# lzzcd001/MeshDiffusion

Hardware: NVIDIA H100
Metric: denoising sample-steps/sec at res-64 (4x64^3), uncond_gen PC sampler (higher is better)
Workload: dtype bf16x3

## Files before the change

meshdiffusion_b200/csrc/gemm_host.cu:

```cuda
#include "gemm_host.h"
#include "elementwise.cuh"
#include <cstring>
#include <cstdlib>
#include <mutex>

namespace mdb {

typedef CUresult (*PFN_encodeTiled)(CUtensorMap*, CUtensorMapDataType, cuuint32_t, void*, const cuuint64_t*,
                                    const cuuint64_t*, const cuuint32_t*, const cuuint32_t*, CUtensorMapInterleave,
                                    CUtensorMapSwizzle, CUtensorMapL2promotion, CUtensorMapFloatOOBfill);

static PFN_encodeTiled get_encode() {
  static PFN_encodeTiled fn = nullptr;
  static std::once_flag once;
  std::call_once(once, [] {
    void* f = nullptr;
    cudaDriverEntryPointQueryResult q;
    cudaError_t e = cudaGetDriverEntryPoint("cuTensorMapEncodeTiled", &f, cudaEnableDefault, &q);
    if (e != cudaSuccess || q != cudaDriverEntryPointSuccess || !f)
      throw std::runtime_error("mdb: cuTensorMapEncodeTiled not available (needs an sm_90+ driver)");
    fn = reinterpret_cast<PFN_encodeTiled>(f);
  });
  return fn;
}
// ... 193 lines not shown
  p.ocs = 1;
  p.kb_elems = kb_elems(prec);
}

void GemmOp::set_output(Precision pr, int X, int Y, int Z, int B, int N, void* out, long long ldc, bool out_fp32) {
  set_output_strided(pr, X, Y, Z, B, N, out, ldc, ldc * X, ldc * X * Y, ldc * X * Y * Z, out_fp32);
}

MapDesc act_map(const Act& a, Precision prec, int part, Geometry box, int sub, int px, int py, int pz) {
  const long long es = esize(prec);
  const long long sx = a.row() * parts(prec) * es, sy = sx * a.X, sz = sy * a.Y, sb = sz * a.Z;
  MapDesc m;
  m.rank = 5;
  m.base = static_cast<char*>(a.ptr) + (long long)part * a.row() * es + px * sx + py * sy + pz * sz;
  m.dims[0] = a.C; m.dims[1] = (a.X - px + sub - 1) / sub; m.dims[2] = (a.Y - py + sub - 1) / sub;
  m.dims[3] = (a.Z - pz + sub - 1) / sub; m.dims[4] = a.B;
  m.strides[0] = sx * sub; m.strides[1] = sy * sub; m.strides[2] = sz * sub; m.strides[3] = sb;
  m.box[0] = kb_elems(prec); m.box[1] = box.bx; m.box[2] = box.by; m.box[3] = box.bz; m.box[4] = box.bb;
  return m;
}

int GemmOp::add_amap(const Act& a, int halo, int sub, int px, int py, int pz, int part) {
  if ((int)amaps_.size() >= kMaxAMaps) throw std::runtime_error("mdb: too many A tensor maps");
  if (halo > 0 && (geo.bz != 1 || geo.bb != 1)) throw std::runtime_error("mdb: halo needs a (bx,by,1,1) tile");
  amaps_.push_back(act_map(a, prec, part, {geo.bx, geo.by + halo, geo.bz, geo.bb}, sub, px, py, pz));
  return (int)amaps_.size() - 1;
}

void GemmOp::add_load_x(int tm_hi, int tm_lo, int nk, int rows, int jrows, int dx, int dy, int dz, int c0, int wsrc,
                        int wc0, int tap0, int tapj) {
  if ((int)loads.size() >= kMaxLoads) throw std::runtime_error("mdb: load table overflow");
  if (rows > kAStageRows) throw std::runtime_error("mdb: A box exceeds the stage size");
  LoadEntry e{};
  e.tmap = (uint8_t)tm_hi; e.tmap_lo = (uint8_t)(prec == kBF16X3 ? tm_lo : tm_hi);
  e.nk = (uint8_t)nk; e.rows = (uint8_t)rows; e.jrows = (uint8_t)jrows;
  e.dx = (int8_t)dx; e.dy = (int8_t)dy; e.dz = (int8_t)dz; e.wsrc = (uint8_t)wsrc;
  e.c0 = (uint16_t)c0; e.wc0 = (uint16_t)wc0; e.tap0 = (uint8_t)tap0; e.tapj = (uint8_t)tapj;
  loads.push_back(e);
  ksteps += nk;
}

void GemmOp::add_conv(const std::vector<Act>& srcs, const float* w, int k, int stride) {
  int ctot = 0;
  for (auto& s : srcs) ctot += s.C;
  const int T = k * k * k;
  add_conv_w(srcs, WSrc{w, 1LL * ctot * T, (long long)T, 1, ctot}, k, stride);
}

void GemmOp::add_conv_dgrad(const Act& dy, const float* w_oidhw, int cin_total, int k) {
  const int T = k * k * k;
  add_conv_w({dy}, WSrc{w_oidhw + (T - 1), (long long)T, 1LL * cin_total * T, -1, dy.C}, k, 1);
}

void GemmOp::add_conv_w(const std::vector<Act>& srcs, const WSrc& wsrc, int k, int stride) {
  const int KB = kb_elems(prec);
  int ctot = 0;
  for (auto& s : srcs) ctot += s.C;
  const int T = k * k * k;
  const int ws = add_wsrc(wsrc);
  const int pad = k / 2;
  flops += 2.0 * p.X * p.Y * p.Z * p.Bn * (double)p.N * ctot * T;
  int coff = 0;
  if (stride == 1) {
    const bool reuse = geo.bz == 1 && geo.bb == 1 && geo.bx * (geo.by + k - 1) <= kAStageRows && p.Y >= geo.by;
    const bool x3 = prec == kBF16X3;
    for (auto& s : srcs) {
      const int tm = add_amap(s, reuse ? k - 1 : 0);
      const int tl = x3 ? add_amap(s, reuse ? k - 1 : 0, 1, 0, 0, 0, 1) : tm;
      for (int c0 = 0; c0 < s.C; c0 += KB) {
        if (reuse) {
          for (int dz = 0; dz < k; ++dz)
            for (int dx = 0; dx < k; ++dx)
              add_load_x(tm, tl, k, geo.bx * (geo.by + k - 1), geo.bx, dx - pad, -pad, dz - pad, c0, ws, coff + c0,
                         (dz * k) * k + dx, k);
        } else {
          for (int dz = 0; dz < k; ++dz)
            for (int dy = 0; dy < k; ++dy)
              for (int dx = 0; dx < k; ++dx)
                add_load_x(tm, tl, 1, kBlockM, 0, dx - pad, dy - pad, dz - pad, c0, ws, coff + c0, (dz * k + dy) * k + dx, 0);
        }
      }
      coff += s.C;
    }
  } else if (stride == 2) {
    if (k != 3) throw std::runtime_error("mdb: stride-2 conv supports k=3 only");
    const bool x3 = prec == kBF16X3;
    for (auto& s : srcs) {
      int tm[8], tl[8];
      for (int par = 0; par < 8; ++par) tm[par] = add_amap(s, 0, 2, par & 1, (par >> 1) & 1, (par >> 2) & 1);
      for (int par = 0; par < 8; ++par) tl[par] = x3 ? add_amap(s, 0, 2, par & 1, (par >> 1) & 1, (par >> 2) & 1, 1) : tm[par];
      for (int c0 = 0; c0 < s.C; c0 += KB)
        for (int dz = 0; dz < 3; ++dz)
          for (int dy = 0; dy < 3; ++dy)
            for (int dx = 0; dx < 3; ++dx) {
              const int par = (dx & 1) | ((dy & 1) << 1) | ((dz & 1) << 2);
              add_load_x(tm[par], tl[par], 1, kBlockM, 0, dx >> 1, dy >> 1, dz >> 1, c0, ws, coff + c0, (dz * 3 + dy) * 3 + dx, 0);
            }
      coff += s.C;
    }
  } else {
    throw std::runtime_error("mdb: unsupported stride");
  }
}

void GemmOp::add_conv_up2(const Act& s, const float* w8, int px, int py, int pz) {
  const int KB = kb_elems(prec);
  const int ws = add_wsrc(WSrc{w8, 8LL * s.C, 8, 1, s.C});
  flops += 2.0 * p.X * p.Y * p.Z * p.Bn * (double)p.N * s.C * 8;
  const bool x3 = prec == kBF16X3;
  const bool reuse = geo.bz == 1 && geo.bb == 1 && geo.bx * (geo.by + 1) <= kAStageRows && p.Y >= geo.by;
  const int tm = add_amap(s, reuse ? 1 : 0);
  const int tl = x3 ? add_amap(s, reuse ? 1 : 0, 1, 0, 0, 0, 1) : tm;
  for (int c0 = 0; c0 < s.C; c0 += KB) {
    for (int ez = 0; ez < 2; ++ez)
      for (int ex = 0; ex < 2; ++ex) {
        if (reuse) {
          add_load_x(tm, tl, 2, geo.bx * (geo.by + 1), geo.bx, ex - 1 + px, -1 + py, ez - 1 + pz, c0, ws, c0, (ez * 2) * 2 + ex, 2);
        } else {
          for (int ey = 0; ey < 2; ++ey)
            add_load_x(tm, tl, 1, kBlockM, 0, ex - 1 + px, ey - 1 + py, ez - 1 + pz, c0, ws, c0, (ez * 2 + ey) * 2 + ex, 0);
        }
      }
  }
}

void GemmOp::add_pointwise(const std::vector<Act>& srcs, const float* w, bool w_in_out) {
  int ctot = 0;
  for (auto& s : srcs) ctot += s.C;
  WSrc ws = w_in_out ? WSrc{w, 1, (long long)p.N, 0, ctot} : WSrc{w, (long long)ctot, 1, 0, ctot};
  add_pointwise_w(srcs, &ws);
}

void GemmOp::add_pointwise_w(const std::vector<Act>& srcs, const WSrc* w) {
  const int KB = kb_elems(prec);
  int ctot = 0;
  for (auto& s : srcs) ctot += s.C;
  int ws = 0;
  if (w) ws = add_wsrc(*w);
  flops += 2.0 * p.X * p.Y * p.Z * p.Bn * (double)p.N * ctot;
  int coff = 0;
  for (auto& s : srcs) {
    const int tm = add_amap(s, 0);
    const int tl = prec == kBF16X3 ? add_amap(s, 0, 1, 0, 0, 0, 1) : tm;
    for (int c0 = 0; c0 < s.C; c0 += KB) add_load_x(tm, tl, 1, kBlockM, 0, 0, 0, 0, c0, ws, coff + c0, 0, 0);
    coff += s.C;
  }
}

void GemmOp::set_residual(const void* res, long long ldr, long long batch_stride, bool fp32) {
  p.res = res;
  p.batch_fastest = batch_stride == 0 ? 1 : 0;
  p.rsx = ldr; p.rsy = ldr * p.X; p.rsz = ldr * p.X * p.Y; p.rsb = batch_stride;
  p.res_fp32 = fp32 ? 1 : 0;
  p.res_lo_off = physical_strides(prec == kBF16X3 && !fp32, ldr, p.rsx, p.rsy, p.rsz, p.rsb);
}

void GemmOp::set_gn_backward(const void* x0, long long ld0, int c0, const void* x1, long long ld1, const void* consts, int silu,
                             float* part) {
  if (prec == kTF32 || p.out_fp32 || p.ocs != 1)
    throw std::runtime_error("mdb: the GroupNorm-backward epilogue is built for bf16 / split-bf16 NDHWC outputs");
  if (p.N % 32 != 0 || (ld1 > 0 && c0 % 32 != 0)) throw std::runtime_error("mdb: GroupNorm-backward epilogue needs 32-channel aligned sources");
  if (splits > 1) throw std::runtime_error("mdb: GroupNorm-backward epilogue cannot be combined with split-K");
  gnb = true;
  p.res = x0; p.res_fp32 = 0; p.batch_fastest = 0;
  p.rsx = ld0; p.rsy = ld0 * p.X; p.rsz = ld0 * p.X * p.Y; p.rsb = ld0 * p.X * p.Y * p.Z;
  p.res1 = x1; p.res_c0 = ld1 > 0 ? c0 : p.N;
  p.r1sx = ld1; p.r1sy = ld1 * p.X; p.r1sz = ld1 * p.X * p.Y; p.r1sb = ld1 * p.X * p.Y * p.Z;
  p.res_lo_off = physical_strides(prec == kBF16X3, ld0, p.rsx, p.rsy, p.rsz, p.rsb);
  p.res1_lo_off = physical_strides(prec == kBF16X3, ld1, p.r1sx, p.r1sy, p.r1sz, p.r1sb);
  p.gnb_c = reinterpret_cast<const float4*>(consts);
  p.gnb_silu = silu;
  p.gnb_part = part;
}

MapDesc GemmOp::b_desc(void* ptr, long long K, int N, int batch, long long rsb, long long bsb) const {
  MapDesc m;
  m.base = ptr; m.rank = 3;
  m.dims[0] = (uint64_t)K; m.dims[1] = (uint64_t)N; m.dims[2] = (uint64_t)batch;
  m.strides[0] = (uint64_t)rsb; m.strides[1] = (uint64_t)bsb;
  m.box[0] = (uint32_t)kb_elems(prec); m.box[1] = (uint32_t)block_n; m.box[2] = 1;
  return m;
}

void GemmOp::set_b_activation(void* ptr, int K, int N, int batch, long long rs, long long bs) {
  b_from_act = true;
  p.b_batched = 1;
  const long long es = esize(prec);
  if (prec == kBF16X3) {
    if (K % kb_elems(prec) != 0) throw std::runtime_error("mdb: X3 activation-B operands need K to be a multiple of 64");
    b_lo_off = rs;
    bmap_ = b_desc(ptr, (int)(rs + K), N, batch, 2 * rs * es, 2 * bs * es);
    return;
  }
  bmap_ = b_desc(ptr, K, N, batch, rs * es, bs * es);
}

struct PackWSrc { const float* ptr; long long sn, sc, st; int cvalid; int ndiv; long long sn_hi; int cdiv; long long sc_hi; };
struct PackArgs { PackWSrc w[4]; };

template <Precision P>
__global__ void __launch_bounds__(256) pack_weights_kernel(const LoadEntry* __restrict__ loads, const int* __restrict__ load_ks0,
                                                         int n_loads, const __grid_constant__ PackArgs args, int N, int ksteps,
                                                         int KB, void* __restrict__ out) {
  const int vpk = KB >> 3;
  const long long total = 1LL * N * n_loads * vpk;
  for (long long idx = blockIdx.x * (long long)blockDim.x + threadIdx.x; idx < total; idx += (long long)gridDim.x * blockDim.x) {
    const int v8 = (int)(idx % vpk);
    const long long t = idx / vpk;
    const int l = (int)(t % n_loads);
    const int n = (int)(t / n_loads);
    const LoadEntry e = loads[l];
    const PackWSrc& w = args.w[e.wsrc];
    const long long noff = w.ndiv ? (long long)(n % w.ndiv) * w.sn + (long long)(n / w.ndiv) * w.sn_hi : (long long)n * w.sn;
    const int c0 = e.wc0 + v8 * 8;
    long long coff[8];
    unsigned valid = 0;
#pragma unroll
    for (int i = 0; i < 8; ++i) {
      const int c = c0 + i;
      if (c < w.cvalid) valid |= 1u << i;
      coff[i] = noff + (w.cdiv ? (long long)(c % w.cdiv) * w.sc + (long long)(c / w.cdiv) * w.sc_hi : (long long)c * w.sc);
    }
    const long long obase = ((long long)n * ksteps + load_ks0[l]) * parts(P) * KB + v8 * 8;
    for (int j = 0; j < e.nk; ++j) {
      const long long toff = (long long)(e.tap0 + j * e.tapj) * w.st;
      float v[8];
#pragma unroll
      for (int i = 0; i < 8; ++i) v[i] = (valid >> i) & 1u ? __ldg(w.ptr + coff[i] + toff) : 0.f;
      ActElem<P>* op = reinterpret_cast<ActElem<P>*>(out) + obase + (long long)j * parts(P) * KB;
      constexpr int E = kVecElems<P>;
#pragma unroll
      for (int i = 0; i < 8 / E; ++i) store_vec<P>(op + E * i, (long long)KB * sizeof(ActElem<P>), v + E * i);
    }
  }
}

void GemmOp::repack(cudaStream_t stream) {
  if (b_from_act) return;
  if (!d_ks0) {
    std::vector<int> ks0;
    int run = 0;
    for (size_t l = 0; l < loads.size(); ++l) { ks0.push_back(run); run += loads[l].nk; }
    if (run != ksteps) throw std::runtime_error("mdb: load table does not cover the packed K extent");
    MDB_CUDA_CHECK(cudaMalloc(&d_ks0, ks0.size() * sizeof(int)));
    MDB_CUDA_CHECK(cudaMemcpy(d_ks0, ks0.data(), ks0.size() * sizeof(int), cudaMemcpyHostToDevice));
  }
  if (wsrcs.size() > 4) throw std::runtime_error("mdb: too many weight sources");
  PackArgs args{};
  for (size_t i = 0; i < wsrcs.size(); ++i) args.w[i] = {wsrcs[i].ptr, wsrcs[i].sn, wsrcs[i].sc, wsrcs[i].st, wsrcs[i].cvalid, wsrcs[i].ndiv, wsrcs[i].sn_hi, wsrcs[i].cdiv, wsrcs[i].sc_hi};
  const int KB = kb_elems(prec), n_loads = (int)loads.size();
  const long long total = 1LL * p.N * n_loads * (KB / 8);
  int blocks = (int)((total + 255) / 256);
  if (blocks > kPlanSMs * 16) blocks = kPlanSMs * 16;
  if (prec == kTF32)
    pack_weights_kernel<kTF32><<<blocks, 256, 0, stream>>>(d_loads, d_ks0, n_loads, args, p.N, ksteps, KB, d_wpacked);
  else if (prec == kBF16X3)
    pack_weights_kernel<kBF16X3><<<blocks, 256, 0, stream>>>(d_loads, d_ks0, n_loads, args, p.N, ksteps, KB, d_wpacked);
  else
    pack_weights_kernel<kBF16><<<blocks, 256, 0, stream>>>(d_loads, d_ks0, n_loads, args, p.N, ksteps, KB, d_wpacked);
  MDB_CUDA_CHECK(cudaGetLastError());
}

void GemmOp::finalize() {
  if (loads.empty()) throw std::runtime_error("mdb: GemmOp without loads");
  p.b_explicit_k = 0;
  p.b_kstep = kb_elems(prec) * parts(prec);
  p.b_lo_k = kb_elems(prec);
  if (b_from_act) p.b_kstep = kb_elems(prec);
  if (b_from_act && prec == kBF16X3) {
    p.b_explicit_k = 1;
    p.b_lo_k = (int)b_lo_off;
  }
  if (!b_from_act) p.b_batched = 0;
  p.n_loads = (int)loads.size();
  if (p.splits < 1) p.splits = 1;
  {
    a_slot_need = 0;
    nk_max = 0;
    p.n_segs = 0;
    p.total_groups = 0;
    size_t i = 0;
    while (i < loads.size()) {
      size_t j = i;
      while (j < loads.size() && loads[j].nk == loads[i].nk && loads[j].rows == loads[i].rows && loads[j].jrows == loads[i].jrows) ++j;
      if (p.n_segs >= kMaxSegs) throw std::runtime_error("mdb: too many pipeline segments");
      GemmSeg sg{};
      sg.n_groups = (int)(j - i); sg.nk = loads[i].nk;
      sg.a_bytes = loads[i].rows * kRowBytes;
      sg.a_stride = (sg.a_bytes + 1023) / 1024 * 1024;
      sg.jbytes = loads[i].jrows * kRowBytes;
      const int need = parts(prec) * sg.a_stride;
      if (sg.a_stride > kAStageBytes) throw std::runtime_error("mdb: A box exceeds the slot size");
      if (need > a_slot_need) a_slot_need = need;
      if (sg.nk > nk_max) nk_max = sg.nk;
      p.segs[p.n_segs++] = sg;
      p.total_groups += sg.n_groups;
      i = j;
    }
  }
  if (p.splits > p.total_groups) { p.splits = p.total_groups; splits = p.splits; }
}

bool GemmOp::epi_tma_ok(const GemmParams& p) const {
  if (gnb || block_n != 128 || prec == kTF32 || p.splits > 1 || p.ocs != 1 || p.out_fp32) return false;
  if (p.res && (p.res_fp32 || p.batch_fastest)) return false;
  const long long es = esize(prec);
  auto aligned = [&](const void* base, long long lo_off, long long sx, long long sy, long long sz, long long sb) {
    const uintptr_t a = reinterpret_cast<uintptr_t>(base);
    return a % 16 == 0 && (lo_off * es) % 16 == 0 && (sx * es) % 16 == 0 && (sy * es) % 16 == 0 && (sz * es) % 16 == 0 &&
           (sb * es) % 16 == 0;
  };
  if (!aligned(p.out, prec == kBF16X3 ? p.out_lo_off : 0, p.osx, p.osy, p.osz, p.osb)) return false;
  if (p.res && !aligned(p.res, prec == kBF16X3 ? p.res_lo_off : 0, p.rsx, p.rsy, p.rsz, p.rsb)) return false;
  return true;
}

static MapDesc epi_map(const void* base, Precision prec, int part, long long lo_off, const GemmParams& q, int B, long long sx,
                       long long sy, long long sz, long long sb) {
  const long long es = esize(prec);
  MapDesc m;
  m.rank = 5;
  m.base = const_cast<char*>(static_cast<const char*>(base)) + (long long)part * lo_off * es;
  m.dims[0] = q.N; m.dims[1] = q.X; m.dims[2] = q.Y; m.dims[3] = q.Z; m.dims[4] = B;
  const long long st[4] = {sx * es, sy * es, sz * es, sb * es};
  long long prev = es * q.N;
  for (int i = 0; i < 4; ++i) {
    m.strides[i] = (uint64_t)(m.dims[i + 1] == 1 ? prev : st[i]);
    prev = (long long)m.strides[i] * (long long)m.dims[i + 1];
  }
  m.box[0] = kRowBytes / es; m.box[1] = q.bx; m.box[2] = q.by; m.box[3] = q.bz; m.box[4] = q.bb;
  return m;
}

void GemmOp::encode_epi_maps(GemmParams& q, int B) const {
  for (int part = 0; part < parts(prec); ++part) {
    encode_map(&q.omap[part], prec, epi_map(q.out, prec, part, q.out_lo_off, q, B, q.osx, q.osy, q.osz, q.osb));
    if (q.res) encode_map(&q.rmap[part], prec, epi_map(q.res, prec, part, q.res_lo_off, q, B, q.rsx, q.rsy, q.rsz, q.rsb));
  }
}

void GemmOp::upload(cudaStream_t stream) {
  for (size_t i = 0; i < amaps_.size(); ++i) encode_map(&p.amap[i], prec, amaps_[i]);
  p.epi_tma = epi_tma_ok(p) ? 1 : 0;
  if (p.epi_tma && p.out) encode_epi_maps(p, p.Bn);
#ifdef MDB_EPI_TRACE
  if (getenv("MDB_EPI_TRACE_PER_THREAD")) p.epi_tma = 0;
  MDB_CUDA_CHECK(cudaMalloc(&d_trace, sizeof(unsigned long long) * kTraceCtas * kTraceTiles * kTraceStamps));
  MDB_CUDA_CHECK(cudaMemset(d_trace, 0, sizeof(unsigned long long) * kTraceCtas * kTraceTiles * kTraceStamps));
  p.trace = d_trace;
  trace_registry().push_back(this);
#endif
  MDB_CUDA_CHECK(cudaMalloc(&d_loads, loads.size() * sizeof(LoadEntry)));
  MDB_CUDA_CHECK(cudaMemcpyAsync(d_loads, loads.data(), loads.size() * sizeof(LoadEntry), cudaMemcpyHostToDevice, stream));
  p.loads = d_loads;
  if (!b_from_act) {
    const long long ktot = 1LL * ksteps * kb_elems(prec) * parts(prec);
    const long long bytes = ktot * p.N * esize(prec);
    MDB_CUDA_CHECK(cudaMalloc(&d_wpacked, bytes));
    owns_w = true;
    bmap_ = b_desc(d_wpacked, ktot, p.N, 1, ktot * esize(prec), bytes);
  }
  encode_map(&p.bmap, prec, bmap_);
  MDB_CUDA_CHECK(cudaStreamSynchronize(stream));
}

void GemmOp::launch(cudaStream_t stream, int B, void* out_override) const {
  GemmParams p = this->p;
  const int smem = pick_slots(p);
  if (B > 0) {
    if (B > this->p.Bn) throw std::runtime_error("mdb: batch exceeds the batch the op was built for");
    p.Bn = B;
    p.tb = (B + p.bb - 1) / p.bb;
  }
  if (out_override) p.out = out_override;
  if (p.epi_tma && (out_override || p.Bn != this->p.Bn)) {
    p.epi_tma = epi_tma_ok(p) ? 1 : 0;
    if (p.epi_tma) encode_epi_maps(p, p.Bn);
  }
  const int tiles_m = p.tx * p.ty * p.tz * p.tb;
  const int total = tiles_m * p.n_tiles_n * (p.splits > 1 ? p.splits : 1);
  const int grid = total < sm_count() ? total : sm_count();
  if (gnb) {
    if (p.splits > 1) throw std::runtime_error("mdb: GroupNorm-backward epilogue: no split-K");
    p.gnb_drop_thresh = rt_drop_thresh; p.gnb_drop_scale = rt_drop_scale; p.gnb_seed = rt_seed;
  }
  gemm_variant(block_n, prec, gnb).launch(p, grid, smem, stream);
  if (p.splits > 1) {
    SplitReduceArgs a{};
    a.partial = p.partial; a.split_stride = p.split_stride; a.splits = p.splits;
    a.bias = p.bias; a.rowbias = p.rowbias; a.rowbias_ld = p.rowbias_ld;
    a.res = p.res; a.res_batch_stride = p.rsb;
    a.out = p.out; a.stats = p.stats; a.voxels = (long long)p.X * p.Y * p.Z; a.N = p.N; a.prec = prec;
    if (prec == kBF16X3) a.res_batch_stride = p.rsb / 2;
    launch_split_reduce(a, p.Bn, stream);
  }
}

}
```

meshdiffusion_b200/csrc/gemm_tc.cuh:

```cuda
#pragma once
#include "ptx.cuh"
#include "act_format.cuh"
#include "gn_stats.cuh"

namespace mdb {

constexpr int kBlockM = 128;
constexpr int kRowBytes = 128;
constexpr int kAStageRows = 160;
constexpr int kAStageBytes = kAStageRows * kRowBytes;
constexpr int kMaxLoads = 2048;
constexpr int kMaxAMaps = 16;
constexpr int kGemmThreads = 384;
constexpr int kEpiThreads = 256;

struct __align__(16) LoadEntry {
  uint8_t tmap;
  uint8_t nk;
  uint8_t rows;
  uint8_t jrows;
  int8_t dx, dy, dz;
  uint8_t wsrc;
  uint16_t c0;
  uint16_t wc0;
  uint8_t tap0;
  uint8_t tapj;
  uint8_t tmap_lo;
  uint8_t pad;
};
static_assert(sizeof(LoadEntry) == 16, "LoadEntry must be 16 bytes");

struct GemmSeg {
  int n_groups;
  int nk;
  int a_bytes;
  int a_stride;
  int jbytes;
};
constexpr int kMaxSegs = 8;

struct GemmParams {
  CUtensorMap amap[kMaxAMaps];
  CUtensorMap bmap;
  CUtensorMap omap[2];
  CUtensorMap rmap[2];
  int epi_tma;
#ifdef MDB_EPI_TRACE
  unsigned long long* trace;
#endif
  const LoadEntry* loads;
  int n_loads;
  int n_segs;
  GemmSeg segs[kMaxSegs];
  int bx, by, bz, bb;
  int X, Y, Z, Bn;
  int tx, ty, tz, tb;
  int n_tiles_n;
  int N;
  int b_batched;
  int splits;
  int total_groups;
  float* partial;
  long long split_stride;
  int batch_fastest;
  int kb_elems;
  int b_explicit_k;
  int b_kstep;
  int b_lo_k;
  int n_aslots, a_slot_bytes, n_bslots, b_slot_bytes;
  long long out_lo_off, res_lo_off;
  void* out;
  long long osx, osy, osz, osb;
  long long ocs;
  int out_fp32;
  const float* bias;
  int bias_on_m;
  const float* rowbias;
  long long rowbias_ld;
  const void* res;
  long long rsx, rsy, rsz, rsb;
  int res_fp32;
  float alpha;
  long long* stats;
  const void* res1;
  long long r1sx, r1sy, r1sz, r1sb;
  long long res1_lo_off;
  int res_c0;
  const float4* gnb_c;
  int gnb_silu;
  int gnb_drop_thresh; float gnb_drop_scale; unsigned long long gnb_seed;
  float* gnb_part;
};

constexpr int kMaxSlots = 8;
constexpr int kMaxDynSmem = 232448;
template <int BLOCK_N, bool kWholeTile = false>
struct GemmCfg {
  static constexpr int kBTileBytes = BLOCK_N * kRowBytes;
  static constexpr int kStatsFloats = 24 * BLOCK_N;
  static constexpr int kStageCols = (kWholeTile || BLOCK_N < 64) ? BLOCK_N : 64;
  static constexpr int kStageRounds = BLOCK_N / kStageCols;
  static_assert(kStageRounds <= 2, "the epilogue stages at most two rounds");
  static constexpr int kAccPitch = kStageCols + 4;
  static constexpr int kAccFloats = kBlockM * kAccPitch;
  static constexpr int kFixedBytes = 1024 + kAccFloats * 4 + kStatsFloats * 4 + 4 * kMaxSlots * 8;
};
constexpr int kRegsProducer = 40, kRegsConsumer = 232;

template <int BLOCK_N, Precision P, bool GNB>
constexpr bool kHasTmaEpi = !GNB && BLOCK_N == 128 && P != kTF32;
constexpr int kEpiBoxBytes = 64 * 2 * kBlockM;
static_assert(kEpiBoxBytes == GemmCfg<128>::kBTileBytes, "an epilogue box is one weight tile");

#ifdef MDB_EPI_TRACE
constexpr int kTraceCtas = 16, kTraceTiles = 64, kTraceStamps = 6;
#define MDB_STAMP(k) do { if (trace_row && et == 0) trace_row[k] = globaltimer(); } while (0)
#else
#define MDB_STAMP(k) do { } while (0)
#endif

__device__ __forceinline__ uint64_t kdesc(uint32_t saddr) { return make_wgmma_desc(saddr, 16, 1024); }

template <int OFF>
__device__ __forceinline__ void colsum_butterfly(float (&s)[32], float (&ss)[32], int lane) {
  const bool hi = (lane & OFF) != 0;
#pragma unroll
  for (int i = 0; i < OFF; ++i) {
    const float send_s = hi ? s[i] : s[i + OFF];
    const float send_q = hi ? ss[i] : ss[i + OFF];
    const float keep_s = hi ? s[i + OFF] : s[i];
    const float keep_q = hi ? ss[i + OFF] : ss[i];
    s[i] = keep_s + __shfl_xor_sync(0xffffffffu, send_s, OFF);
    ss[i] = keep_q + __shfl_xor_sync(0xffffffffu, send_q, OFF);
  }
  if constexpr (OFF > 1) colsum_butterfly<OFF / 2>(s, ss, lane);
}

template <Precision P>
__device__ __forceinline__ void add_res_chunk(const uint4 (&buf)[8], float (&v)[32]) {
  constexpr int E = kVecElems<P>, NV = 32 / E;
#pragma unroll
  for (int i = 0; i < NV; ++i) {
    float r[E];
    decode_vec<P>(buf[i], buf[P == kBF16X3 ? NV + i : i], r);
#pragma unroll
    for (int j = 0; j < E; ++j) v[E * i + j] += r[j];
  }
}

template <int BLOCK_N, Precision P, bool GNB>
__global__ void __launch_bounds__(kGemmThreads, 1) gemm_tc_kernel(const __grid_constant__ GemmParams p) {
  static_assert(!(GNB && P == kTF32), "the GroupNorm-backward epilogue is built for bf16 / split-bf16 operands");
  using Cfg = GemmCfg<BLOCK_N, GNB>;
  constexpr int kParts = parts(P);
  const int NA = p.n_aslots, NB = p.n_bslots;
  const uint32_t a_slot = (uint32_t)p.a_slot_bytes, b_slot = (uint32_t)p.b_slot_bytes;
  extern __shared__ uint8_t smem_raw[];
  uint8_t* smem = reinterpret_cast<uint8_t*>((reinterpret_cast<uintptr_t>(smem_raw) + 1023) & ~uintptr_t(1023));
  float* s_acc = reinterpret_cast<float*>(smem + NA * p.a_slot_bytes + NB * p.b_slot_bytes);
  float* s_stats = s_acc + Cfg::kAccFloats;
  uint64_t* bars = reinterpret_cast<uint64_t*>(s_stats + Cfg::kStatsFloats);

  const uint32_t a_ring = smem_u32(smem), b_ring = a_ring + NA * a_slot;
  const uint32_t a_full = smem_u32(bars), a_empty = a_full + 8 * kMaxSlots;
  const uint32_t b_full = a_empty + 8 * kMaxSlots, b_empty = b_full + 8 * kMaxSlots;

  const int warp = __shfl_sync(0xffffffffu, (int)(threadIdx.x >> 5), 0), lane = threadIdx.x & 31;

  if (warp == 0 && lane == 0) {
    for (int i = 0; i < kMaxAMaps; ++i) tma_prefetch_desc(&p.amap[i]);
    tma_prefetch_desc(&p.bmap);
  }
  if (warp == 1 && lane == 0) {
    for (int i = 0; i < NA; ++i) { mbar_init(a_full + 8 * i, 1); mbar_init(a_empty + 8 * i, 2); }
    for (int i = 0; i < NB; ++i) { mbar_init(b_full + 8 * i, 1); mbar_init(b_empty + 8 * i, 2); }
    fence_barrier_init();
    fence_proxy_async();
  }
  __syncthreads();

  const int tiles_m = p.tx * p.ty * p.tz * p.tb;
  const int splits = p.splits > 1 ? p.splits : 1;
  const int total_tiles = tiles_m * p.n_tiles_n * splits;
  const int first_tile = (int)blockIdx.x;
  const int tile_step = (int)gridDim.x;

  auto split_range = [&](int item, int& lo, int& hi) {
    const int sidx = item % splits;
    lo = (int)((long long)p.total_groups * sidx / splits);
    hi = (int)((long long)p.total_groups * (sidx + 1) / splits);
  };
  int mt_of_tile = 0;
  auto decode = [&](int tile, int& x0, int& y0, int& z0, int& b0, int& n0) {
    tile /= splits;
    int nt = tile % p.n_tiles_n;
    int mt = tile / p.n_tiles_n;
    mt_of_tile = mt;
    n0 = nt * BLOCK_N;
    int bt = 0;
    if (p.batch_fastest) { bt = mt % p.tb; mt /= p.tb; }
    int xt = mt % p.tx; mt /= p.tx;
    int yt = mt % p.ty; mt /= p.ty;
    int zt = mt % p.tz; mt /= p.tz;
    if (!p.batch_fastest) bt = mt;
    x0 = xt * p.bx; y0 = yt * p.by; z0 = zt * p.bz; b0 = bt * p.bb;
  };

  if (warp < 4) {
    setmaxnreg_dec<kRegsProducer>();
    if (warp == 0) {
      uint32_t as = 0, aph = 0, bs = 0, bph = 0;
      for (int tile = first_tile; tile < total_tiles; tile += tile_step) {
        int x0, y0, z0, b0, n0;
        decode(tile, x0, y0, z0, b0, n0);
        int kcol = 0, l = 0, gi = 0, g_lo, g_hi;
        split_range(tile, g_lo, g_hi);
        const int bcoord = p.b_batched ? b0 : 0;
        for (int sg = 0; sg < p.n_segs; ++sg) {
          const GemmSeg& seg = p.segs[sg];
          for (int g = 0; g < seg.n_groups; ++g, ++gi) {
            if (gi < g_lo || gi >= g_hi) {
              kcol += seg.nk * p.b_kstep;
              ++l;
              continue;
            }
            const uint4 raw = __ldg(reinterpret_cast<const uint4*>(p.loads + l));
            const LoadEntry& en = reinterpret_cast<const LoadEntry&>(raw);
            mbar_wait(a_empty + 8 * as, aph ^ 1);
            if (elect_one()) {
              const uint32_t abase = a_ring + as * a_slot, bar = a_full + 8 * as;
              mbar_expect_tx(bar, kParts * seg.a_bytes);
              tma_load_5d(&p.amap[en.tmap], bar, abase, en.c0, x0 + en.dx, y0 + en.dy, z0 + en.dz, b0);
              if constexpr (P == kBF16X3) tma_load_5d(&p.amap[en.tmap_lo], bar, abase + seg.a_stride, en.c0, x0 + en.dx, y0 + en.dy, z0 + en.dz, b0);
            }
            __syncwarp();
            if (++as == (uint32_t)NA) { as = 0; aph ^= 1; }
            int kc = (P == kBF16X3 && p.b_explicit_k) ? (int)en.wc0 : kcol;
            for (int j = 0; j < seg.nk; ++j) {
              mbar_wait(b_empty + 8 * bs, bph ^ 1);
              if (elect_one()) {
                const uint32_t bbase = b_ring + bs * b_slot, bar = b_full + 8 * bs;
                mbar_expect_tx(bar, kParts * Cfg::kBTileBytes);
                tma_load_3d(&p.bmap, bar, bbase, kc, n0, bcoord);
                if constexpr (P == kBF16X3) tma_load_3d(&p.bmap, bar, bbase + Cfg::kBTileBytes, kc + p.b_lo_k, n0, bcoord);
              }
              __syncwarp();
              kc += p.b_kstep;
              if (++bs == (uint32_t)NB) { bs = 0; bph ^= 1; }
            }
            kcol += seg.nk * p.b_kstep;
            ++l;
          }
        }
        if constexpr (kHasTmaEpi<BLOCK_N, P, GNB>) {
          if (p.epi_tma) {
            for (int rnd = 0; rnd < Cfg::kStageRounds; ++rnd) {
              mbar_wait(b_empty + 8 * bs, bph ^ 1);
              if (elect_one()) {
                const uint32_t bbase = b_ring + bs * b_slot, bar = b_full + 8 * bs;
                const int c = n0 + rnd * Cfg::kStageCols;
                if (p.res && c < p.N) {
                  mbar_expect_tx(bar, kParts * kEpiBoxBytes);
                  tma_load_5d(&p.rmap[0], bar, bbase, c, x0, y0, z0, b0);
                  if constexpr (P == kBF16X3) tma_load_5d(&p.rmap[1], bar, bbase + kEpiBoxBytes, c, x0, y0, z0, b0);
                } else {
                  mbar_arrive(bar);
                }
              }
              __syncwarp();
              if (++bs == (uint32_t)NB) { bs = 0; bph ^= 1; }
            }
          }
        }
      }
    }
  } else {
    setmaxnreg_inc<kRegsConsumer>();
    const int wg = (warp - 4) >> 2;
    const int wt = threadIdx.x & 127;
    const int q = warp & 3;
    const int half = (warp - 4) >> 2;
    constexpr int kChunks = BLOCK_N / 32;
    constexpr int kChunkStep = kChunks >= 2 ? 2 : 1;
    const int row = q * 32 + lane;
    const int et = threadIdx.x - 128;
    const int rows_per_b = p.bx * p.by * p.bz;
    const int seg = row / rows_per_b;
    int it = 0;
    int staged_n0 = -1, staged_b0 = -1, bias_buf = 0;
    int want_cols = 0;
    if constexpr (GNB) {
      want_cols = (p.stats != nullptr || p.gnb_part != nullptr) ? 1 : 0;
      asm volatile("" : "+r"(want_cols));
    }
    uint32_t as = 0, aph = 0, bs = 0, bph = 0;
    int epi_pend = -1;
    for (int tile = first_tile; tile < total_tiles; tile += tile_step, ++it) {
      const int vit = it;
#ifdef MDB_EPI_TRACE
      unsigned long long* trace_row = (p.trace && (int)blockIdx.x < kTraceCtas && it < kTraceTiles)
                                          ? p.trace + ((long long)blockIdx.x * kTraceTiles + it) * kTraceStamps : nullptr;
      bool first_k = true;
#endif
      if constexpr (kHasTmaEpi<BLOCK_N, P, GNB>) {
        if (et == 0 && epi_pend >= 0) {
          bulk_wait_read<0>();
          mbar_arrive(b_empty + 8 * epi_pend);
          mbar_arrive(b_empty + 8 * epi_pend);
          epi_pend = -1;
        }
      }
      constexpr int kAccRegs = kParts * BLOCK_N / 2;
      float acc[kAccRegs];
      float (&acc_hi)[BLOCK_N / 2] = *reinterpret_cast<float (*)[BLOCK_N / 2]>(acc);
#pragma unroll
      for (int i = 0; i < kAccRegs; ++i) acc[i] = 0.f;
      {
        int gi = 0, g_lo, g_hi;
        split_range(tile, g_lo, g_hi);
        int prev_b = -1, prev_a = -1;
        const uint32_t a_row0 = (uint32_t)wg * 64 * kRowBytes;
        for (int sg = 0; sg < p.n_segs; ++sg) {
          const GemmSeg& sgm = p.segs[sg];
          for (int g = 0; g < sgm.n_groups; ++g, ++gi) {
            if (gi < g_lo || gi >= g_hi) continue;
            mbar_wait(a_full + 8 * as, aph);
            const uint32_t abase = a_ring + as * a_slot + a_row0;
            for (int j = 0; j < sgm.nk; ++j) {
              mbar_wait(b_full + 8 * bs, bph);
#ifdef MDB_EPI_TRACE
              if (first_k) { MDB_STAMP(5); first_k = false; }
#endif
              const uint64_t ad = kdesc(abase + j * sgm.jbytes);
              const uint64_t bd = kdesc(b_ring + bs * b_slot);
              wgmma_fence();
              if constexpr (P == kBF16X3) {
                const uint64_t adl = kdesc(abase + sgm.a_stride + j * sgm.jbytes);
#pragma unroll
                for (int k = 0; k < kRowBytes / 32; ++k) wgmma_kmajor<2 * BLOCK_N, false>(acc, ad + 2 * k, bd + 2 * k, 1u);
                wgmma_fence();
#pragma unroll
                for (int k = 0; k < kRowBytes / 32; ++k) wgmma_kmajor<BLOCK_N, false>(acc_hi, adl + 2 * k, bd + 2 * k, 1u);
              } else {
#pragma unroll
                for (int k = 0; k < kRowBytes / 32; ++k) wgmma_kmajor<BLOCK_N, P == kTF32>(acc, ad + 2 * k, bd + 2 * k, 1u);
              }
              wgmma_commit();
              wgmma_wait<1>();
              if (wt == 0) {
                if (prev_b >= 0) mbar_arrive(b_empty + 8 * prev_b);
                if (prev_a >= 0) mbar_arrive(a_empty + 8 * prev_a);
              }
              prev_b = (int)bs;
              prev_a = j + 1 == sgm.nk ? (int)as : -1;
              if (++bs == (uint32_t)NB) { bs = 0; bph ^= 1; }
            }
            if (++as == (uint32_t)NA) { as = 0; aph ^= 1; }
          }
        }
        wgmma_wait<0>();
        fence_operands(acc);
        MDB_STAMP(0);
        if (wt == 0) {
          if (prev_b >= 0) mbar_arrive(b_empty + 8 * prev_b);
          if (prev_a >= 0) mbar_arrive(a_empty + 8 * prev_a);
        }
        if constexpr (P == kBF16X3) {
#pragma unroll
          for (int i = 0; i < BLOCK_N / 2; ++i) acc[i] += acc[BLOCK_N / 2 + i];
        }
      }
      int x0, y0, z0, b0, n0;
      decode(tile, x0, y0, z0, b0, n0);
      int r = row;
      const int xl = r % p.bx; r /= p.bx;
      const int yl = r % p.by; r /= p.by;
      const int zl = r % p.bz; r /= p.bz;
      const int xg = x0 + xl, yg = y0 + yl, zg = z0 + zl, bg = b0 + r;
      const bool valid = (xg < p.X) && (yg < p.Y) && (zg < p.Z) && (bg < p.Bn);
      const long long ooff = xg * p.osx + yg * p.osy + zg * p.osz + bg * p.osb;
      const long long roff = xg * p.rsx + yg * p.rsy + zg * p.rsz + bg * p.rsb;

      constexpr int kRoundRegs = Cfg::kStageCols / 2;
      auto stage = [&]() {
        const int w4 = (warp & 3), srow = wg * 64 + w4 * 16 + (lane >> 2), scol = 2 * (lane & 3);
#pragma unroll
        for (int j = 0; j < Cfg::kStageCols / 8; ++j) {
          *reinterpret_cast<float2*>(s_acc + srow * Cfg::kAccPitch + 8 * j + scol) = make_float2(acc[4 * j], acc[4 * j + 1]);
          *reinterpret_cast<float2*>(s_acc + (srow + 8) * Cfg::kAccPitch + 8 * j + scol) = make_float2(acc[4 * j + 2], acc[4 * j + 3]);
        }
      };
      named_bar_sync(2, kEpiThreads);
      stage();
      if constexpr (Cfg::kStageRounds > 1) {
#pragma unroll
        for (int i = 0; i < kRoundRegs; ++i) acc[i] = acc[kRoundRegs + i];
      }

      const int bkey = p.rowbias ? b0 : 0;
      if (n0 != staged_n0 || bkey != staged_b0) {
        staged_n0 = n0; staged_b0 = bkey;
        bias_buf ^= 1;
        float* wb = s_stats + 16 * BLOCK_N + bias_buf * 4 * BLOCK_N;
        for (int i = et; i < p.bb * BLOCK_N; i += kEpiThreads) {
          const int sg = i / BLOCK_N, c = i % BLOCK_N;
          const int n = n0 + c, bgl = b0 + sg;
          float bv = 0.f;
          if (n < p.N) {
            if (p.bias && !p.bias_on_m) bv += __ldg(p.bias + n);
            if (p.rowbias && bgl < p.Bn) bv += __ldg(p.rowbias + static_cast<long long>(bgl) * p.rowbias_ld + n);
          }
          wb[i] = bv;
        }
      }
      const float* s_bias = s_stats + 16 * BLOCK_N + bias_buf * 4 * BLOCK_N;
      float* s_part = s_stats + (vit & 1) * 8 * BLOCK_N;
      uint4 rbuf[8];
      auto prefetch_res = [&](int ch) {
        const int nbp = n0 + ch * 32;
        if (!(p.res && valid && p.ocs == 1 && nbp + 32 <= p.N)) return;
        if constexpr (GNB) {
          const bool second = p.res1 && nbp >= p.res_c0;
          const __nv_bfloat16* base = reinterpret_cast<const __nv_bfloat16*>(second ? p.res1 : p.res);
          const long long off = second ? xg * p.r1sx + yg * p.r1sy + zg * p.r1sz + bg * p.r1sb + (nbp - p.res_c0) : roff + nbp;
          const uint4* rp = reinterpret_cast<const uint4*>(base + off);
#pragma unroll
          for (int i = 0; i < 4; ++i) rbuf[i] = __ldg(rp + i);
          if constexpr (P == kBF16X3) {
            const uint4* rl = reinterpret_cast<const uint4*>(base + off + (second ? p.res1_lo_off : p.res_lo_off));
#pragma unroll
            for (int i = 0; i < 4; ++i) rbuf[4 + i] = __ldg(rl + i);
          }
          return;
        }
        if (P == kTF32 || p.res_fp32) {
          const uint4* rp = reinterpret_cast<const uint4*>(reinterpret_cast<const float*>(p.res) + roff + nbp);
#pragma unroll
          for (int i = 0; i < 8; ++i) rbuf[i] = __ldg(rp + i);
        } else {
          const uint4* rp = reinterpret_cast<const uint4*>(reinterpret_cast<const __nv_bfloat16*>(p.res) + roff + nbp);
#pragma unroll
          for (int i = 0; i < 4; ++i) rbuf[i] = __ldg(rp + i);
          if constexpr (P == kBF16X3) {
            const uint4* rl = reinterpret_cast<const uint4*>(reinterpret_cast<const __nv_bfloat16*>(p.res) + roff + nbp + p.res_lo_off);
#pragma unroll
            for (int i = 0; i < 4; ++i) rbuf[4 + i] = __ldg(rl + i);
          }
        }
      };
      const bool tma_epi = kHasTmaEpi<BLOCK_N, P, GNB> && p.epi_tma != 0;
      const int ch0 = kChunkStep == 2 ? half : 0;
      const bool active = kChunkStep == 2 || half == 0;
      if (active && !tma_epi) prefetch_res(ch0);

      constexpr int kRoundChunks = Cfg::kStageCols / 32;
#pragma unroll 1
      for (int rnd = 0; rnd < Cfg::kStageRounds; ++rnd) {
        if (rnd > 0) {
          named_bar_sync(2, kEpiThreads);
          stage();
        }
        named_bar_sync(2, kEpiThreads);
        if (rnd == 0) MDB_STAMP(1);
        int eslot_i = 0;
        uint8_t* eslot = nullptr;
        if constexpr (kHasTmaEpi<BLOCK_N, P, GNB>) {
          if (tma_epi) {
            eslot_i = (int)bs;
            eslot = smem + NA * p.a_slot_bytes + bs * p.b_slot_bytes;
            mbar_wait(b_full + 8 * bs, bph);
            if (++bs == (uint32_t)NB) { bs = 0; bph ^= 1; }
          }
        }

#pragma unroll 1
        for (int ch = ch0 + rnd * kRoundChunks; ch < (rnd + 1) * kRoundChunks && active; ch += kChunkStep) {
          uint32_t rr[32];
          {
            const float4* src = reinterpret_cast<const float4*>(s_acc + row * Cfg::kAccPitch + (ch - rnd * kRoundChunks) * 32);
#pragma unroll
            for (int i = 0; i < 8; ++i) {
              const float4 t = src[i];
              rr[4 * i] = __float_as_uint(t.x); rr[4 * i + 1] = __float_as_uint(t.y);
              rr[4 * i + 2] = __float_as_uint(t.z); rr[4 * i + 3] = __float_as_uint(t.w);
            }
          }
          const int nb = n0 + ch * 32;
          if (nb >= p.N) continue;
          if (splits > 1) {
            if (valid) {
              float* pp = p.partial + (long long)(tile % splits) * p.split_stride + (P == kBF16X3 ? (ooff >> 1) : ooff) + nb;
              if (nb + 32 <= p.N) {
#pragma unroll
                for (int i = 0; i < 8; ++i)
                  reinterpret_cast<float4*>(pp)[i] = make_float4(__uint_as_float(rr[4 * i]), __uint_as_float(rr[4 * i + 1]),
                                                                 __uint_as_float(rr[4 * i + 2]), __uint_as_float(rr[4 * i + 3]));
              } else {
                for (int i = 0; i < 32; ++i) if (nb + i < p.N) pp[i] = __uint_as_float(rr[i]);
              }
            }
            continue;
          }
          const bool full = (nb + 32 <= p.N) && (p.ocs == 1);
          float v[32];
          const float mbias = (p.bias && p.bias_on_m && valid) ? __ldg(p.bias + xg) : 0.f;
          const float* sb = s_bias + (seg < 4 ? seg : 0) * BLOCK_N + ch * 32;
#pragma unroll
          for (int i = 0; i < 32; ++i) v[i] = __uint_as_float(rr[i]) * p.alpha + mbias + sb[i];
          float q2[GNB ? 32 : 1];
          if constexpr (GNB) {
            if (valid) {
              const float4* cc = p.gnb_c + static_cast<long long>(bg) * p.N + nb;
              unsigned long long hsh[8];
              if (p.gnb_drop_thresh > 0) {
                const unsigned long long e4 = (unsigned long long)((((static_cast<long long>(bg) * p.Z + zg) * p.Y + yg) * p.X + xg) * p.N + nb) >> 2;
#pragma unroll
                for (int i = 0; i < 8; ++i) hsh[i] = drop_hash64(p.gnb_seed, e4 + i);
              }
#pragma unroll
              for (int i = 0; i < 32; ++i) {
                const float4 kc = __ldg(cc + i);
                const __nv_bfloat16 xb = reinterpret_cast<const __nv_bfloat16*>(rbuf)[i];
                float xv = __bfloat162float(xb);
                if constexpr (P == kBF16X3) xv += __bfloat162float(reinterpret_cast<const __nv_bfloat16*>(rbuf + 4)[i]);
                float d = v[i];
                if (p.gnb_drop_thresh > 0) {
                  const unsigned r16 = (unsigned)((hsh[i >> 2] >> (16 * (i & 3))) & 0xFFFFu);
                  d = r16 >= (unsigned)p.gnb_drop_thresh ? d * p.gnb_drop_scale : 0.f;
                }
                if (p.gnb_silu) {
                  const float h = fmaf(xv, kc.x, kc.y);
                  d *= P == kBF16X3 ? dsilu_ex2_half(h) : dsilu_tanh_half(h);
                }
                v[i] = d;
                q2[i] = d * fmaf(xv, kc.z, kc.w);
              }
            } else {
#pragma unroll
              for (int i = 0; i < 32; ++i) q2[i] = 0.f;
            }
          }
          const int chr = ch - rnd * kRoundChunks;
          auto eoff = [&](int i) { return row * 128 + (((4 * chr + i) ^ (row & 7)) << 4); };
          if (!GNB && p.res && valid && tma_epi) {
            uint4 buf[8];
#pragma unroll
            for (int i = 0; i < 4; ++i) {
              buf[i] = *reinterpret_cast<const uint4*>(eslot + eoff(i));
              buf[4 + i] = P == kBF16X3 ? *reinterpret_cast<const uint4*>(eslot + kEpiBoxBytes + eoff(i)) : buf[i];
            }
            add_res_chunk<P>(buf, v);
          } else if (!GNB && p.res && valid) {
            if (P == kTF32 || p.res_fp32) {
              if (full) {
                add_res_chunk<kTF32>(rbuf, v);
              } else {
                const float* rp = reinterpret_cast<const float*>(p.res) + roff + nb;
                for (int i = 0; i < 32; ++i) if (nb + i < p.N) v[i] += rp[i];
              }
            } else {
              if (full) {
                add_res_chunk<P>(rbuf, v);
              } else {
                const ActElem<P>* rp = reinterpret_cast<const ActElem<P>*>(p.res) + roff + nb;
                for (int i = 0; i < 32; ++i) if (nb + i < p.N) v[i] += load_split<P>(rp + i, p.res_lo_off);
              }
            }
          }
          if (!tma_epi && ch + kChunkStep < kChunks) prefetch_res(ch + kChunkStep);
          if (tma_epi) {
#pragma unroll
            for (int i = 0; i < 4; ++i) {
              const uint4 h = bf16x8_encode(v + 8 * i);
              *reinterpret_cast<uint4*>(eslot + eoff(i)) = h;
              if constexpr (P == kBF16X3) *reinterpret_cast<uint4*>(eslot + kEpiBoxBytes + eoff(i)) = bf16x8_encode_lo(h, v + 8 * i);
            }
          } else if (valid) {
            if (p.out_fp32) {
              float* op = reinterpret_cast<float*>(p.out) + ooff + nb;
              if (full) {
#pragma unroll
                for (int i = 0; i < 8; ++i) reinterpret_cast<float4*>(op)[i] = make_float4(v[4 * i], v[4 * i + 1], v[4 * i + 2], v[4 * i + 3]);
              } else {
                for (int i = 0; i < 32; ++i) if (nb + i < p.N) op[i * p.ocs] = v[i];
              }
            } else {
              ActElem<P>* op = reinterpret_cast<ActElem<P>*>(p.out) + ooff + nb;
              if (full) {
                constexpr int E = kVecElems<P>;
#pragma unroll
                for (int i = 0; i < 32 / E; ++i) store_vec<P>(op + E * i, p.out_lo_off * (long long)sizeof(ActElem<P>), v + E * i);
              } else {
                for (int i = 0; i < 32; ++i) if (nb + i < p.N) store_split<P>(op + i * p.ocs, p.out_lo_off, v[i]);
              }
            }
          }
          if (GNB ? (want_cols != 0) : (p.stats != nullptr)) {
            float s[32], ss[32];
#pragma unroll
            for (int i = 0; i < 32; ++i) {
              const float t = valid ? v[i] : 0.f;
              s[i] = t; ss[i] = GNB ? q2[GNB ? i : 0] : t * t;
            }
            colsum_butterfly<16>(s, ss, lane);
            s_part[(q * 2 + 0) * BLOCK_N + ch * 32 + lane] = s[0];
            s_part[(q * 2 + 1) * BLOCK_N + ch * 32 + lane] = ss[0];
          }
        }
        if constexpr (kHasTmaEpi<BLOCK_N, P, GNB>) {
          if (tma_epi) {
            fence_proxy_async();
            named_bar_sync(2, kEpiThreads);
            if (et == 0) {
              const int c = n0 + rnd * Cfg::kStageCols;
              const uint32_t src = b_ring + eslot_i * b_slot;
              if (c < p.N) {
                tma_store_5d(&p.omap[0], src, c, x0, y0, z0, b0);
                if constexpr (P == kBF16X3) tma_store_5d(&p.omap[1], src + kEpiBoxBytes, c, x0, y0, z0, b0);
              }
              bulk_commit();
              if (epi_pend >= 0) {
                bulk_wait_read<1>();
                mbar_arrive(b_empty + 8 * epi_pend);
                mbar_arrive(b_empty + 8 * epi_pend);
              }
              epi_pend = eslot_i;
            }
          }
        }
        MDB_STAMP(2 + rnd);
      }
      if constexpr (GNB) {
        if (p.gnb_part && splits == 1) {
          named_bar_sync(1, kEpiThreads);
          const int warps_per_seg = rows_per_b >= 128 ? 4 : rows_per_b / 32;
          for (int i = et; i < p.bb * BLOCK_N; i += kEpiThreads) {
            const int sg = i / BLOCK_N, c = i % BLOCK_N;
            const int n = n0 + c;
            if (mt_of_tile < tiles_m && n < p.N) {
              float ts = 0.f, tq = 0.f;
              for (int w = sg * warps_per_seg; w < (sg + 1) * warps_per_seg; ++w) {
                ts += s_part[(w * 2 + 0) * BLOCK_N + c];
                tq += s_part[(w * 2 + 1) * BLOCK_N + c];
              }
              float* dst = p.gnb_part + ((static_cast<long long>(mt_of_tile) * p.bb + sg) * p.N + n) * 2;
              dst[0] = ts; dst[1] = tq;
            }
          }
        }
      }
      if (!GNB && p.stats && splits == 1) {
        named_bar_sync(1, kEpiThreads);
        const int warps_per_seg = rows_per_b >= 128 ? 4 : rows_per_b / 32;
        for (int i0 = 0; i0 < p.bb * BLOCK_N; i0 += kEpiThreads) {
          const int i = i0 + et;
          const int sg = i / BLOCK_N, c = i % BLOCK_N;
          const int bgl = b0 + sg, n = n0 + c;
          if (i < p.bb * BLOCK_N && bgl < p.Bn && n < p.N) {
            float ts = 0.f, tq = 0.f;
            for (int w = sg * warps_per_seg; w < (sg + 1) * warps_per_seg; ++w) {
              ts += s_part[(w * 2 + 0) * BLOCK_N + c];
              tq += s_part[(w * 2 + 1) * BLOCK_N + c];
            }
            long long* dst = p.stats + (static_cast<long long>(bgl) * p.N + n) * kStatWords;
            stat_add(dst, ts);
            stat_add(dst + 2, tq);
          }
        }
      }
      MDB_STAMP(4);
    }
    if constexpr (kHasTmaEpi<BLOCK_N, P, GNB>) {
      if (et == 0 && epi_pend >= 0) bulk_wait<0>();
    }
  }
}

}
```

Before: 37.89.

## Extend TMA epilogue stores to fp32 outputs and defer epilogue slot release

Allows the TMA-store epilogue path for fp32 outputs under bf16x3 precision. It writes swizzled fp32 boxes into shared memory and encodes two fp32 tensor maps of 32 columns each, replacing per-thread global stores. It also moves the wait-and-release of the previous epilogue buffer from the start of each tile into the producer-consumer k-loop, adds a fast path in split_range for a single split, and vectorises the bias loads. The intent is to overlap output stores with the next tile's main loop and cut uncoalesced epilogue traffic, at the cost of more complex slot lifetimes and swizzle-correctness risk.

```diff
diff --git a/meshdiffusion_b200/csrc/gemm_host.cu b/meshdiffusion_b200/csrc/gemm_host.cu
--- a/meshdiffusion_b200/csrc/gemm_host.cu
+++ b/meshdiffusion_b200/csrc/gemm_host.cu
@@ -519,16 +519,18 @@
 }
 
 bool GemmOp::epi_tma_ok(const GemmParams& p) const {
-  if (gnb || block_n != 128 || prec == kTF32 || p.splits > 1 || p.ocs != 1 || p.out_fp32) return false;
+  if (gnb || block_n != 128 || prec == kTF32 || p.splits > 1 || p.ocs != 1) return false;
+  if (p.out_fp32 && (prec != kBF16X3 || p.res)) return false;
   if (p.res && (p.res_fp32 || p.batch_fastest)) return false;
-  const long long es = esize(prec);
-  auto aligned = [&](const void* base, long long lo_off, long long sx, long long sy, long long sz, long long sb) {
+  auto aligned = [&](const void* base, long long es, long long lo_off, long long sx, long long sy, long long sz, long long sb) {
     const uintptr_t a = reinterpret_cast<uintptr_t>(base);
     return a % 16 == 0 && (lo_off * es) % 16 == 0 && (sx * es) % 16 == 0 && (sy * es) % 16 == 0 && (sz * es) % 16 == 0 &&
            (sb * es) % 16 == 0;
   };
-  if (!aligned(p.out, prec == kBF16X3 ? p.out_lo_off : 0, p.osx, p.osy, p.osz, p.osb)) return false;
-  if (p.res && !aligned(p.res, prec == kBF16X3 ? p.res_lo_off : 0, p.rsx, p.rsy, p.rsz, p.rsb)) return false;
+  if (p.out_fp32) return aligned(p.out, 4, 0, p.osx, p.osy, p.osz, p.osb);
+  const long long es = esize(prec);
+  if (!aligned(p.out, es, prec == kBF16X3 ? p.out_lo_off : 0, p.osx, p.osy, p.osz, p.osb)) return false;
+  if (p.res && !aligned(p.res, es, prec == kBF16X3 ? p.res_lo_off : 0, p.rsx, p.rsy, p.rsz, p.rsb)) return false;
   return true;
 }
 
@@ -550,6 +552,14 @@
 }
 
 void GemmOp::encode_epi_maps(GemmParams& q, int B) const {
+  if (q.out_fp32) {
+    for (int part = 0; part < 2; ++part) {
+      MapDesc m = epi_map(q.out, kTF32, part, 32, q, B, q.osx, q.osy, q.osz, q.osb);
+      m.dims[0] = q.N - 32 * part;
+      encode_map(&q.omap[part], kTF32, m);
+    }
+    return;
+  }
   for (int part = 0; part < parts(prec); ++part) {
     encode_map(&q.omap[part], prec, epi_map(q.out, prec, part, q.out_lo_off, q, B, q.osx, q.osy, q.osz, q.osb));
     if (q.res) encode_map(&q.rmap[part], prec, epi_map(q.res, prec, part, q.res_lo_off, q, B, q.rsx, q.rsy, q.rsz, q.rsb));
diff --git a/meshdiffusion_b200/csrc/gemm_tc.cuh b/meshdiffusion_b200/csrc/gemm_tc.cuh
--- a/meshdiffusion_b200/csrc/gemm_tc.cuh
+++ b/meshdiffusion_b200/csrc/gemm_tc.cuh
@@ -111,6 +111,8 @@
 constexpr bool kHasTmaEpi = !GNB && BLOCK_N == 128 && P != kTF32;
 constexpr int kEpiBoxBytes = 64 * 2 * kBlockM;
 static_assert(kEpiBoxBytes == GemmCfg<128>::kBTileBytes, "an epilogue box is one weight tile");
+template <Precision P>
+constexpr bool kTmaF32Out = P == kBF16X3;
 
 #ifdef MDB_EPI_TRACE
 constexpr int kTraceCtas = 16, kTraceTiles = 64, kTraceStamps = 6;
@@ -156,7 +158,7 @@
   const int NA = p.n_aslots, NB = p.n_bslots;
   const uint32_t a_slot = (uint32_t)p.a_slot_bytes, b_slot = (uint32_t)p.b_slot_bytes;
   extern __shared__ uint8_t smem_raw[];
-  uint8_t* smem = reinterpret_cast<uint8_t*>((reinterpret_cast<uintptr_t>(smem_raw) + 1023) & ~uintptr_t(1023));
+  uint8_t* smem = smem_raw + ((1024u - (smem_u32(smem_raw) & 1023u)) & 1023u);
   float* s_acc = reinterpret_cast<float*>(smem + NA * p.a_slot_bytes + NB * p.b_slot_bytes);
   float* s_stats = s_acc + Cfg::kAccFloats;
   uint64_t* bars = reinterpret_cast<uint64_t*>(s_stats + Cfg::kStatsFloats);
@@ -186,6 +188,7 @@
   const int tile_step = (int)gridDim.x;
 
   auto split_range = [&](int item, int& lo, int& hi) {
+    if (splits == 1) { lo = 0; hi = p.total_groups; return; }
     const int sidx = item % splits;
     lo = (int)((long long)p.total_groups * sidx / splits);
     hi = (int)((long long)p.total_groups * (sidx + 1) / splits);
@@ -302,14 +305,6 @@
                                           ? p.trace + ((long long)blockIdx.x * kTraceTiles + it) * kTraceStamps : nullptr;
       bool first_k = true;
 #endif
-      if constexpr (kHasTmaEpi<BLOCK_N, P, GNB>) {
-        if (et == 0 && epi_pend >= 0) {
-          bulk_wait_read<0>();
-          mbar_arrive(b_empty + 8 * epi_pend);
-          mbar_arrive(b_empty + 8 * epi_pend);
-          epi_pend = -1;
-        }
-      }
       constexpr int kAccRegs = kParts * BLOCK_N / 2;
       float acc[kAccRegs];
       float (&acc_hi)[BLOCK_N / 2] = *reinterpret_cast<float (*)[BLOCK_N / 2]>(acc);
@@ -351,6 +346,14 @@
                 if (prev_b >= 0) mbar_arrive(b_empty + 8 * prev_b);
                 if (prev_a >= 0) mbar_arrive(a_empty + 8 * prev_a);
               }
+              if constexpr (kHasTmaEpi<BLOCK_N, P, GNB>) {
+                if (epi_pend >= 0) {
+                  bulk_wait_read<0>();
+                  mbar_arrive(b_empty + 8 * epi_pend);
+                  mbar_arrive(b_empty + 8 * epi_pend);
+                  epi_pend = -1;
+                }
+              }
               prev_b = (int)bs;
               prev_a = j + 1 == sgm.nk ? (int)as : -1;
               if (++bs == (uint32_t)NB) { bs = 0; bph ^= 1; }
@@ -504,9 +507,15 @@
           const bool full = (nb + 32 <= p.N) && (p.ocs == 1);
           float v[32];
           const float mbias = (p.bias && p.bias_on_m && valid) ? __ldg(p.bias + xg) : 0.f;
-          const float* sb = s_bias + (seg < 4 ? seg : 0) * BLOCK_N + ch * 32;
-#pragma unroll
-          for (int i = 0; i < 32; ++i) v[i] = __uint_as_float(rr[i]) * p.alpha + mbias + sb[i];
+          const float4* sb = reinterpret_cast<const float4*>(s_bias + (seg < 4 ? seg : 0) * BLOCK_N + ch * 32);
+#pragma unroll
+          for (int i = 0; i < 8; ++i) {
+            const float4 b = sb[i];
+            v[4 * i] = __uint_as_float(rr[4 * i]) * p.alpha + mbias + b.x;
+            v[4 * i + 1] = __uint_as_float(rr[4 * i + 1]) * p.alpha + mbias + b.y;
+            v[4 * i + 2] = __uint_as_float(rr[4 * i + 2]) * p.alpha + mbias + b.z;
+            v[4 * i + 3] = __uint_as_float(rr[4 * i + 3]) * p.alpha + mbias + b.w;
+          }
           float q2[GNB ? 32 : 1];
           if constexpr (GNB) {
             if (valid) {
@@ -568,7 +577,12 @@
             }
           }
           if (!tma_epi && ch + kChunkStep < kChunks) prefetch_res(ch + kChunkStep);
-          if (tma_epi) {
+          if (tma_epi && kTmaF32Out<P> && p.out_fp32) {
+            uint8_t* box = eslot + chr * kEpiBoxBytes + row * 128;
+#pragma unroll
+            for (int i = 0; i < 8; ++i)
+              *reinterpret_cast<float4*>(box + ((i ^ (row & 7)) << 4)) = make_float4(v[4 * i], v[4 * i + 1], v[4 * i + 2], v[4 * i + 3]);
+          } else if (tma_epi) {
 #pragma unroll
             for (int i = 0; i < 4; ++i) {
               const uint4 h = bf16x8_encode(v + 8 * i);
@@ -616,7 +630,8 @@
               const uint32_t src = b_ring + eslot_i * b_slot;
               if (c < p.N) {
                 tma_store_5d(&p.omap[0], src, c, x0, y0, z0, b0);
-                if constexpr (P == kBF16X3) tma_store_5d(&p.omap[1], src + kEpiBoxBytes, c, x0, y0, z0, b0);
+                if (P == kBF16X3 && !(kTmaF32Out<P> && p.out_fp32 && c + 32 >= p.N))
+                  tma_store_5d(&p.omap[1], src + kEpiBoxBytes, c, x0, y0, z0, b0);
               }
               bulk_commit();
               if (epi_pend >= 0) {
```

Measured after the change: 38.43 (median of 6 runs). 1.4% higher.
